# bootphon/shennong

Hardware: AMD Instinct MI355X
Metric: frames/s (25 ms/10 ms, 16 kHz) for fbank-40 + MFCC-13 at 1/2/4/8 GPUs (higher is better)
Workload: dtype f32

## Files before the change

### include/shennong_amd.h

```cpp
#ifndef SHENNONG_AMD_H_
#define SHENNONG_AMD_H_

#include <stdint.h>

#ifdef __cplusplus
extern "C" {
#endif

#define SNF_OK 0
#define SNF_E_INVALID (-1)
#define SNF_E_RUNTIME (-2)
#define SNF_E_HIP (-3)
#define SNF_E_NODEVICE (-4)

#define SNF_KIND_SPECTROGRAM 0
#define SNF_KIND_FBANK 1
#define SNF_KIND_MFCC 2
#define SNF_KIND_PLP 3
#define SNF_KIND_PITCH 4
#define SNF_KIND_PITCH_POST 5
#define SNF_KIND_DELTA 6
#define SNF_KIND_ENERGY 7
#define SNF_KIND_VAD 8
#define SNF_KIND_CMVN 9
// ... 295 lines not shown
int snf_memcpy_h2d_async(void* dst, const void* src, uint64_t bytes, void* stream);
int snf_memcpy_d2h_async(void* dst, const void* src, uint64_t bytes, void* stream);
int snf_event_create(void** event);
int snf_event_destroy(void* event);
int snf_event_record(void* event, void* stream);
int snf_event_synchronize(void* event);
int snf_stream_wait_event(void* stream, void* event);
int snf_event_elapsed_ms(void* start, void* stop, float* ms);
int snf_host_malloc(void** hptr, uint64_t bytes);
int snf_host_free(void* hptr);
int snf_wav_scan(const char* path, int32_t* channels, int32_t* sample_rate, int64_t* nsamples, int32_t* bits,
                 int32_t* format_tag);
int snf_wav_read_pcm16(const char* const* paths, int64_t n_files, const int64_t* first_sample,
                       const int64_t* n_samples, int16_t* dst, const int64_t* dst_offsets, int32_t threads,
                       int32_t* status);

#define SNF_COMM_ID_BYTES 128
typedef struct snf_comm snf_comm;
int snf_comm_unique_id(void* id128);
int snf_comm_init(const void* id128, int32_t world_size, int32_t rank, int32_t device_id, snf_comm** out);
int snf_comm_rank(const snf_comm* comm);
int snf_comm_world_size(const snf_comm* comm);
int snf_comm_destroy(snf_comm* comm);
int snf_comm_gatherv(snf_comm* comm, const float* d_send, int64_t send_count, float* d_recv,
                     const int64_t* recv_counts, int32_t root, void* stream);
int snf_comm_allreduce_f64(snf_comm* comm, double* d_buf, int64_t count, int32_t op, void* stream);

int snf_debug_fill_lds(uint32_t pattern);
int snf_debug_pitch_scratch(snf_plan* plan, void** down, void** nccf_res, void** pov_nccf,
                            void** states);
int snf_debug_plp_tail(snf_plan* plan, const float* mel, const double* energy,
                       const int64_t* frame_offsets, int64_t n_utts, float* out, float* mel_out);
int snf_debug_fbank512b_rel32(const int64_t* sample_offsets, const int64_t* frame_offsets, int64_t n_utts);
float snf_plan_last_kernel_ms(const snf_plan* plan, int which);
const char* snf_plan_kernel_name(const snf_plan* plan, int which);

#ifdef __cplusplus
}
#endif
#endif
```

### shennong_amd/_backend.py

```python

import ctypes as C
import os
import threading

import numpy as np

from shennong_amd import _abi

_HERE = os.path.dirname(os.path.abspath(__file__))
_LIB_PATH = os.environ.get('SHENNONG_AMD_LIB') or os.path.join(_HERE, 'libshennong_hip.so')
_LIB = None
_LOCK = threading.Lock()
_PLANS = {}
_DEVICE = int(os.environ.get('SHENNONG_AMD_DEVICE', '0'))

EXPORTS = [
    'snf_version', 'snf_last_error', 'snf_device_count', 'snf_set_device',
    'snf_device_name', 'snf_device_synchronize', 'snf_num_frames',
    'snf_first_sample_of_frame', 'snf_window_size', 'snf_window_shift',
    'snf_padded_window_size', 'snf_window_function', 'snf_pitch_num_frames',
    'snf_plan_create', 'snf_plan_destroy', 'snf_plan_ndims', 'snf_plan_fast_path',
    'snf_plan_num_frames', 'snf_plan_run_batch', 'snf_plan_run_batch_device',
    'snf_post_ndims', 'snf_post_run_batch', 'snf_post_run_batch_device',
    'snf_cmvn_accumulate', 'snf_cmvn_apply', 'snf_cmvn_accumulate_device',
    'snf_cmvn_apply_device', 'snf_concat_columns_device', 'snf_count_nonfinite_device', 'snf_set_noise_call',
    'snf_malloc', 'snf_free', 'snf_memcpy_h2d', 'snf_memcpy_d2h', 'snf_memset',
    'snf_host_malloc', 'snf_host_free', 'snf_debug_fill_lds', 'snf_debug_pitch_scratch',
    'snf_debug_plp_tail', 'snf_debug_fbank512b_rel32',
    'snf_stream_create', 'snf_stream_destroy', 'snf_stream_synchronize', 'snf_memcpy_h2d_async',
    'snf_memcpy_d2h_async', 'snf_comm_unique_id', 'snf_comm_init', 'snf_comm_rank', 'snf_comm_world_size',
    'snf_comm_destroy', 'snf_comm_gatherv', 'snf_comm_allreduce_f64',
    'snf_plan_last_kernel_ms', 'snf_plan_kernel_name', 'snf_set_oom_hook',
    'snf_event_create', 'snf_event_destroy', 'snf_event_record', 'snf_event_elapsed_ms', 'snf_mem_info',
    'snf_stream_wait_event', 'snf_stream_query', 'snf_event_synchronize', 'snf_wav_scan', 'snf_wav_read_pcm16',
    'snf_gmm_loglikes', 'snf_gmm_accumulate', 'snf_gmm_gselect', 'snf_gmm_gselect_preselect',
    'snf_gmm_selection_posteriors', 'snf_fmllr_accumulate', 'snf_vtln_gram', 'snf_lvtln_select',
    'snf_affine_apply_segments', 'snf_vtln_gram_rows', 'snf_dense_layer', 'snf_bottleneck_vad',
    'snf_bottleneck_fbank', 'snf_bottleneck_nn_input', 'snf_bottleneck_forward', 'snf_crepe_conv',
    'snf_crepe_forward', 'snf_crepe_decode', 'snf_framed_onehot', 'snf_packed_weights_bf16_size',
    'snf_pack_weights_bf16', 'snf_dense_layer_bf16', 'snf_bottleneck_forward_bf16', 'snf_crepe_conv_bf16',
    'snf_crepe_forward_bf16', 'snf_resample_num_out', 'snf_linear_resample', 'snf_crepe_rows',
    'snf_crepe_voicing_convert', 'snf_bottleneck_extract', 'snf_bottleneck_extract_runs',
    'snf_collate_num_out', 'snf_collate_padded', 'snf_dtw_pairs']


_OOM_HOOK_TYPE = C.CFUNCTYPE(None)


def _release_pool():
    try:
        DEVICE_POOL.clear()
    except Exception:
        pass


_OOM_HOOK = _OOM_HOOK_TYPE(_release_pool)


def lib():
    global _LIB
    if _LIB is not None:
# ... 34 lines not shown
        L.snf_plan_fast_path.argtypes = [vp]
        L.snf_plan_num_frames.argtypes = [vp, i64]
        L.snf_plan_num_frames.restype = i64
        L.snf_plan_run_batch.argtypes = [vp, pi16, pi64, i64, pf, pf, pi64]
        L.snf_plan_run_batch_device.argtypes = [
            vp, vp, pi64, i64, pf, vp, pi64, vp]
        L.snf_post_ndims.argtypes = [vp, i32]
        L.snf_post_run_batch.argtypes = [vp, pf, i32, pi64, i64, pf]
        L.snf_post_run_batch_device.argtypes = [vp, vp, i32, pi64, i64, vp, vp]
        pi32, pf64 = C.POINTER(C.c_int32), C.POINTER(C.c_double)
        L.snf_cmvn_accumulate.argtypes = [
            vp, pf, i32, pi64, i64, pf, pi32, i32, pf64]
        L.snf_cmvn_apply.argtypes = [
            vp, pf, i32, pi64, i64, pf64, pi32, i32, i32, i32, pf]
        L.snf_cmvn_accumulate_device.argtypes = [
            vp, vp, i32, pi64, i64, vp, pi32, i32, pf64]
        L.snf_cmvn_apply_device.argtypes = [
            vp, vp, i32, pi64, i64, pf64, pi32, i32, i32, i32, vp]
        L.snf_concat_columns_device.argtypes = [
            i32, vp, i32, pi64, vp, i32, pi64, i64, vp, pi64]
        L.snf_count_nonfinite_device.argtypes = [i32, vp, C.c_uint64, C.POINTER(C.c_uint64)]
        L.snf_set_noise_call.argtypes = [C.c_uint64]
        L.snf_malloc.argtypes = [C.POINTER(vp), C.c_uint64]
        L.snf_free.argtypes = [vp]
        L.snf_memcpy_h2d.argtypes = [vp, vp, C.c_uint64]
        L.snf_memcpy_d2h.argtypes = [vp, vp, C.c_uint64]
        L.snf_memset.argtypes = [vp, i32, C.c_uint64]
        L.snf_host_malloc.argtypes = [C.POINTER(vp), C.c_uint64]
        L.snf_host_free.argtypes = [vp]
        L.snf_debug_fill_lds.argtypes = [C.c_uint32]
        L.snf_debug_pitch_scratch.argtypes = [vp] + [C.POINTER(vp)] * 4
        L.snf_debug_plp_tail.argtypes = [vp, pf, C.POINTER(C.c_double), pi64, i64, pf, pf]
        L.snf_debug_fbank512b_rel32.argtypes = [pi64, pi64, i64]
        L.snf_stream_create.argtypes = [C.POINTER(vp)]
        L.snf_stream_destroy.argtypes = [vp]
        L.snf_stream_synchronize.argtypes = [vp]
        L.snf_stream_query.argtypes = [vp]
        L.snf_memcpy_h2d_async.argtypes = [vp, vp, C.c_uint64, vp]
        L.snf_event_create.argtypes = [C.POINTER(vp)]
        L.snf_event_destroy.argtypes = [vp]
        L.snf_event_record.argtypes = [vp, vp]
        L.snf_stream_wait_event.argtypes = [vp, vp]
        L.snf_event_synchronize.argtypes = [vp]
        L.snf_event_elapsed_ms.argtypes = [vp, vp, C.POINTER(C.c_float)]
        L.snf_memcpy_d2h_async.argtypes = [vp, vp, C.c_uint64, vp]
        L.snf_comm_unique_id.argtypes = [vp]
        L.snf_comm_init.argtypes = [vp, i32, i32, i32, C.POINTER(vp)]
        L.snf_comm_rank.argtypes = [vp]
        L.snf_comm_world_size.argtypes = [vp]
        L.snf_comm_destroy.argtypes = [vp]
        L.snf_comm_gatherv.argtypes = [vp, vp, i64, vp, pi64, i32, vp]
        L.snf_comm_allreduce_f64.argtypes = [vp, vp, i64, i32, vp]
        L.snf_plan_last_kernel_ms.argtypes = [vp, i32]
        L.snf_plan_last_kernel_ms.restype = f32
        L.snf_plan_kernel_name.argtypes = [vp, i32]
        L.snf_plan_kernel_name.restype = C.c_char_p
        L.snf_set_oom_hook.argtypes = [_OOM_HOOK_TYPE]
        L.snf_mem_info.argtypes = [C.POINTER(C.c_uint64), C.POINTER(C.c_uint64)]
        L.snf_wav_scan.argtypes = [C.c_char_p, pi32, pi32, pi64, pi32, pi32]
        L.snf_wav_read_pcm16.argtypes = [C.POINTER(C.c_char_p), i64, pi64, pi64, pi16, pi64, i32, pi32]
        L.snf_gmm_loglikes.argtypes = [i32, vp, i64, i32, vp, vp, vp, i32, vp, vp]
        L.snf_gmm_accumulate.argtypes = [i32, vp, i64, i32, vp, vp, vp, vp, i32, vp, vp, vp, vp]
        L.snf_gmm_gselect.argtypes = [i32, vp, i64, i32, vp, vp, vp, i32, i32, vp, vp, vp]
        L.snf_gmm_gselect_preselect.argtypes = [i32, vp, i64, i32, vp, vp, vp, i32, vp, i32, i32, vp, vp, vp]
        L.snf_gmm_selection_posteriors.argtypes = [i32, vp, i64, i32, vp, vp, vp, i32, vp, i32, f32, vp, vp, vp]
        L.snf_fmllr_accumulate.argtypes = [i32, vp, i64, i32, vp, vp, i32, vp, vp, i32, vp, i64, vp, vp]
# ... 1251 lines not shown
```

### shennong_amd/csrc/capi_mel.hip

```cpp
#include "plan.h"

using namespace snf;

namespace {

constexpr float kPairSplitRatio = 8.0f;

int check_offsets(const snf_plan* plan, const int64_t* sample_offsets, const int64_t* frame_offsets,
                  int64_t n_utts) {
  if (sample_offsets[0] != 0 || frame_offsets[0] != 0)
    return set_error(SNF_E_INVALID, "offsets tables must start at 0");
  for (int64_t u = 0; u < n_utts; ++u) {
    const int64_t n = sample_offsets[u + 1] - sample_offsets[u];
    const int64_t f = frame_offsets[u + 1] - frame_offsets[u];
    if (n < 0 || f < 0) return set_error(SNF_E_INVALID, "offsets tables must be non-decreasing");
    if (f != snf_plan_num_frames(plan, n))
      return set_error(SNF_E_INVALID, "frame_offsets do not match snf_plan_num_frames for utterance " +
                                          std::to_string(u));
  }
  return SNF_OK;
}

int run_pitch_device(snf_plan* plan, const int16_t* d_wave, const int64_t* sample_offsets,
                     int64_t n_utts, float* d_out, const int64_t* frame_offsets, hipStream_t s) {
// ... 446 lines not shown
  const size_t nb = static_cast<size_t>(plan->o.mel.num_bins), nc = static_cast<size_t>(plan->ndims);
  DevBuf d_mel, d_energy, d_foff, d_out;
  if ((rc = d_mel.ensure(sizeof(float) * nf * nb))) return rc;
  if ((rc = d_energy.ensure(sizeof(double) * nf))) return rc;
  if ((rc = d_out.ensure(sizeof(float) * nf * nc))) return rc;
  if ((rc = d_foff.upload(std::vector<int64_t>(frame_offsets, frame_offsets + n_utts + 1), s))) return rc;
  SNF_HIP_CHECK(hipMemcpyAsync(d_mel.p, mel, sizeof(float) * nf * nb, hipMemcpyHostToDevice, s));
  SNF_HIP_CHECK(hipMemcpyAsync(d_energy.p, energy, sizeof(double) * nf, hipMemcpyHostToDevice, s));
  BatchArgs b{};
  b.frame_offsets = d_foff.as<int64_t>();
  b.n_utts = n_utts;
  b.total_frames = total_frames;
  begin_timing(plan);
  if (plan->o.rasta) {
    if ((rc = launch_rasta(d_mel.as<float>(), b, static_cast<int>(nb), s))) return rc;
    mark_kernel(plan, "rasta_kernel");
  }
  const char* launched = nullptr;
  rc = launch_plp_tail(plan->pp, b, d_mel.as<float>(), d_energy.as<double>(), d_out.as<float>(), s, &launched);
  if (!rc && launched) mark_kernel(plan, launched);
  if (!rc) {
    SNF_HIP_CHECK(hipMemcpyAsync(out, d_out.p, sizeof(float) * nf * nc, hipMemcpyDeviceToHost, s));
    if (mel_out) SNF_HIP_CHECK(hipMemcpyAsync(mel_out, d_mel.p, sizeof(float) * nf * nb, hipMemcpyDeviceToHost, s));
  }
  SNF_HIP_CHECK(hipStreamSynchronize(s));
  return rc;
}

int snf_debug_fbank512b_rel32(const int64_t* sample_offsets, const int64_t* frame_offsets, int64_t n_utts) {
  if (!sample_offsets || !frame_offsets || n_utts < 0) return set_error(SNF_E_INVALID, "null offsets table");
  return fbank512b_rel32_ok(sample_offsets, frame_offsets, n_utts) ? 1 : 0;
}

}
```

### shennong_amd/csrc/device_fft.h

```cpp
#ifndef SNF_DEVICE_FFT_H_
#define SNF_DEVICE_FFT_H_

#include <float.h>
#include <hip/hip_runtime.h>

#include <cstdint>

namespace snf {

namespace {

__device__ __forceinline__ float fast_log(float x) {
  return __builtin_amdgcn_logf(x) * 0.69314718055994530942f;
}
__device__ __forceinline__ float floor_eps(float x) {
  return __builtin_amdgcn_fmed3f(x, FLT_EPSILON, FLT_MAX);
}
template <int SHIFT>
__device__ __forceinline__ void fmac_row_shl(float& acc, float src, float f) {
  asm volatile("s_nop 1\n v_fmac_f32_dpp %0, %1, %2 row_shl:%3 row_mask:0xf bank_mask:0xf bound_ctrl:1"
               : "+v"(acc) : "v"(src), "v"(f), "n"(SHIFT));
}

typedef __attribute__((address_space(3))) const void* lds_cptr;
__device__ __forceinline__ unsigned lds_addr(const void* p) {
  return static_cast<unsigned>(reinterpret_cast<uintptr_t>((lds_cptr)p));
}
__device__ __forceinline__ void lds_wait() {
  asm volatile("s_waitcnt lgkmcnt(0)" ::: "memory");
  __builtin_amdgcn_sched_barrier(0);
}
__device__ __forceinline__ void read16_b64(const void* base, float2 (&d)[16]) {
  asm volatile(
      "ds_read_b64 %0, %16\n ds_read_b64 %1, %16 offset:8\n ds_read_b64 %2, %16 offset:16\n"
      "ds_read_b64 %3, %16 offset:24\n ds_read_b64 %4, %16 offset:32\n ds_read_b64 %5, %16 offset:40\n"
      "ds_read_b64 %6, %16 offset:48\n ds_read_b64 %7, %16 offset:56\n ds_read_b64 %8, %16 offset:64\n"
      "ds_read_b64 %9, %16 offset:72\n ds_read_b64 %10, %16 offset:80\n ds_read_b64 %11, %16 offset:88\n"
      "ds_read_b64 %12, %16 offset:96\n ds_read_b64 %13, %16 offset:104\n ds_read_b64 %14, %16 offset:112\n"
      "ds_read_b64 %15, %16 offset:120\n s_waitcnt lgkmcnt(0)"
      : "=&v"(d[0]), "=&v"(d[1]), "=&v"(d[2]), "=&v"(d[3]), "=&v"(d[4]), "=&v"(d[5]), "=&v"(d[6]),
        "=&v"(d[7]), "=&v"(d[8]), "=&v"(d[9]), "=&v"(d[10]), "=&v"(d[11]), "=&v"(d[12]), "=&v"(d[13]),
        "=&v"(d[14]), "=&v"(d[15])
      : "v"(lds_addr(base))
      : "memory");
}
__device__ __forceinline__ void read_tw8_row16(const void* tw, const void* base, float4 (&q)[8], float2 (&d)[16]) {
  asm volatile(
      "ds_read_b128 %0, %24\n ds_read_b128 %1, %24 offset:16\n ds_read_b128 %2, %24 offset:32\n"
      "ds_read_b128 %3, %24 offset:48\n ds_read_b128 %4, %24 offset:64\n ds_read_b128 %5, %24 offset:80\n"
      "ds_read_b128 %6, %24 offset:96\n ds_read_b128 %7, %24 offset:112\n"
      "ds_read_b64 %8, %25\n ds_read_b64 %9, %25 offset:8\n ds_read_b64 %10, %25 offset:16\n"
      "ds_read_b64 %11, %25 offset:24\n ds_read_b64 %12, %25 offset:32\n ds_read_b64 %13, %25 offset:40\n"
      "ds_read_b64 %14, %25 offset:48\n ds_read_b64 %15, %25 offset:56\n ds_read_b64 %16, %25 offset:64\n"
      "ds_read_b64 %17, %25 offset:72\n ds_read_b64 %18, %25 offset:80\n ds_read_b64 %19, %25 offset:88\n"
// ... 303 lines not shown
```

### shennong_amd/csrc/kernels_fbank512b.hip

```cpp
#include <float.h>

#include <cstdlib>
#include <type_traits>

#include "snf_internal.h"
#include "device_fft.h"

namespace snf {

namespace {

typedef unsigned u32x4 __attribute__((ext_vector_type(4)));
typedef unsigned u32x2 __attribute__((ext_vector_type(2)));

constexpr int kWaves = kFast512MaxWaves;
constexpr int kHeaderFloats = kFast512HeaderFloats;
constexpr int kTileRow = kFast512TileRow;
constexpr int kTileBytes = kFast512TileBytes;


}

template <int NJ, int KIND, int ENERGY, bool BST, bool DITHER, int MMQ, int LV, bool REL>
__global__ __launch_bounds__(kWaves * 64, 4) void fbank512b_kernel(const Fast512Params p, const BatchArgs b,
// ... 17 lines not shown
  float2* tile = reinterpret_cast<float2*>(wave_base);
  float* ptile = reinterpret_cast<float*>(wave_base) + q * 16;
  tile[l * kTileRow + 16] = make_float2(0.0f, 0.0f);
  const int mj = lane & 3;
  const float* __restrict__ mm_lane = tab + p.off_mm_lane + lane;
  const float* __restrict__ mtile =
      reinterpret_cast<const float*>(smem + tab_bytes + (wid * 4 + mj) * kTileBytes) + mj * 16;
  int mm_start_once = 0, mm_out_once = 0;
  if (NJ == 13) {
    mm_start_once = reinterpret_cast<const int*>(mm_lane)[0];
    mm_out_once = reinterpret_cast<const int*>(mm_lane)[64];
  }
  static_assert(MMQ == 0 || (NJ == 13 && (MMQ == 6 || MMQ == 7) && (LV == 3 || LV == 4)), "plans of launch_plan");
  const float4* __restrict__ mm_b_once = reinterpret_cast<const float4*>(mtile + mm_start_once);
  float lifter_once = 1.0f;
  if (NJ == 13 && KIND == SNF_KIND_MFCC) lifter_once = t_lifter[l];

  const float win_len_f = static_cast<float>(p.win_len), inv_win_len = 1.0f / win_len_f;
  using idx_t = typename std::conditional<REL, int, int64_t>::type;
  const idx_t total_frames = static_cast<idx_t>(b.total_frames);
  const idx_t n_sets = (total_frames + 3) >> 2;
  const idx_t set_stride = static_cast<idx_t>(gridDim.x) * kWaves;
  const idx_t last_frame = total_frames - 1;
  idx_t set = static_cast<idx_t>(blockIdx.x) * kWaves + wid;
  if (set >= n_sets) return;

  const bool in_last = 2 * (l + 16 * (NJ - 1)) < p.win_len;
  auto in_window = [&](int j) -> bool {
    if (NJ == 13) return j < NJ - 1 || in_last;
    return 2 * (l + 16 * j) < p.win_len;
  };
  static_assert(!REL || NJ == 13, "set-relative addressing: the 25 ms forms");
  const unsigned q8 = static_cast<unsigned>(q) * 8u;
  auto set_rows_of = [&](const void* table, idx_t s) -> uint64_t {
    int rows = static_cast<int>(total_frames) - static_cast<int>(s) * 4;
    rows = rows < 0 ? 0 : rows;
    asm volatile("" : "+s"(rows));
    rows = rows > 4 ? 4 : rows;
    const __amdgpu_buffer_rsrc_t rsrc = __builtin_amdgcn_make_buffer_rsrc(
        const_cast<char*>(static_cast<const char*>(table)) + static_cast<int64_t>(s) * 32, 0, rows * 8, 0x00020000);
    const u32x2 v = __builtin_amdgcn_raw_buffer_load_b64(rsrc, q8, 0, 0);
    return (static_cast<uint64_t>(v.y) << 32) | v.x;
  };
  auto start_of = [&](idx_t s) -> int64_t {
    if (REL) return static_cast<int64_t>(set_rows_of(b.frame_start, s));
    const int64_t gi = s * 4 + q;
    return b.frame_start[gi < last_frame ? gi : last_frame];
  };
  auto noise_of = [&](idx_t s) -> unsigned long long {
    if (!DITHER) return 0ull;
    if (REL) return set_rows_of(b.frame_noise, s);
    const int64_t gi = s * 4 + q;
    return b.frame_noise[gi < last_frame ? gi : last_frame];
  };
  typedef int __attribute__((aligned(2))) int_a2;
  int raw[NJ];
  const unsigned l4 = 4u * l, off12 = in_last ? l4 + 64u * 12u : 0u;
  auto request = [&](int64_t st) {
    if (REL) {
      const unsigned lo = static_cast<unsigned>(st), hi = static_cast<unsigned>(static_cast<uint64_t>(st) >> 32);
      const unsigned lo0 = __builtin_amdgcn_readfirstlane(lo), hi0 = __builtin_amdgcn_readfirstlane(hi);
      const int64_t st0 = static_cast<int64_t>((static_cast<uint64_t>(hi0) << 32) | lo0);
      const int64_t left = b.rel32_samples - st0;
      unsigned over = static_cast<unsigned>(static_cast<uint64_t>(left) >> 31);
      asm volatile("" : "+s"(over));
      const __amdgpu_buffer_rsrc_t wrsrc = __builtin_amdgcn_make_buffer_rsrc(
          const_cast<int16_t*>(b.wave + st0), 0, over != 0u ? -1 : static_cast<int>(static_cast<unsigned>(left) << 1),
          0x00020000);
      unsigned off = ((lo - lo0) << 1) + l4, last = ((lo - lo0) << 1) + off12;
      asm volatile("" : "+v"(off), "+v"(last));
#pragma unroll
      for (int j = 0; j < NJ - 1; ++j)
        raw[j] = static_cast<int>(__builtin_amdgcn_raw_buffer_load_b32(wrsrc, off + 64u * j, 0, 0));
      raw[NJ - 1] = static_cast<int>(__builtin_amdgcn_raw_buffer_load_b32(wrsrc, last, 0, 0));
      return;
    }
    const int16_t* __restrict__ wp = b.wave + st;
    const int16_t* __restrict__ wl = wp + 2 * l;
#pragma unroll
    for (int j = 0; j < NJ; ++j)
      raw[j] = *reinterpret_cast<const int_a2*>((NJ == 13 && j < NJ - 1) || in_window(j) ? wl + 32 * j : wp);
  };
  float4 w512q[4];
  read_quads<4>(t_tw512 + l * 10, w512q);
  int64_t start_next = start_of(set + set_stride);
  unsigned long long noise_cur = noise_of(set), noise_next = noise_of(set + set_stride);
  request(start_of(set));
  if (BST) {
    const __amdgpu_buffer_rsrc_t none = __builtin_amdgcn_make_buffer_rsrc(out, 0, 0, 0x00020000);
    if (KIND == SNF_KIND_MFCC) __builtin_amdgcn_raw_buffer_store_b32(0u, none, -1, 0, 0);
    else __builtin_amdgcn_raw_buffer_store_b128(u32x4{0u, 0u, 0u, 0u}, none, -1, 0, 2);
  }

  for (; set < n_sets; set += set_stride) {
    const idx_t g = set * 4 + q;
    const bool valid = g <= last_frame;

    float xe[NJ], xo[NJ];
    int part_i = 0;
    float part = 0.0f;
    unsigned dkey_lo = 0, dkey_hi = 0;
    if (DITHER) {
      const unsigned long long k = noise_cur ^ p.seed;
      dkey_lo = fmix32(static_cast<unsigned>(k));
      dkey_hi = fmix32(static_cast<unsigned>(k >> 32) ^ dkey_lo);
      asm volatile("" : "+v"(dkey_lo), "+v"(dkey_hi));
    }
    const float dscale = DITHER ? dither_scale(p.dither) : 0.0f;
#pragma unroll
    for (int j = 0; j < NJ; ++j) {
      xe[j] = static_cast<float>(static_cast<short>(raw[j] & 0xffff));
      xo[j] = static_cast<float>(raw[j] >> 16);
      if (DITHER) {
        add_dither_pair(dkey_lo, dkey_hi, static_cast<unsigned>(l + 16 * j), dscale, xe[j], xo[j]);
        const float s2 = xe[j] + xo[j];
        part += in_window(j) ? s2 : 0.0f;
      } else {
        const int both = __builtin_amdgcn_sdot2(__builtin_bit_cast(short2v, raw[j]), short2v{1, 1}, part_i, false);
        part_i = in_window(j) ? both : part_i;
      }
    }
    if (!DITHER) part = static_cast<float>(part_i);
#pragma unroll
    for (int j = 0; j < NJ; ++j) asm volatile("" : "+v"(xe[j]), "+v"(xo[j]) : : "memory");
    asm volatile("" : "+v"(part) : : "memory");
    request(start_next);
    start_next = start_of(set + 2 * set_stride);
    if (DITHER) {
      noise_cur = noise_next;
      noise_next = noise_of(set + 2 * set_stride);
    }

    float neg_mean = 0.0f;
    if (p.remove_dc) {
      const float sum = row_sum16(part);
      const float qv = sum * inv_win_len;
      neg_mean = -__builtin_fmaf(__builtin_fmaf(-qv, win_len_f, sum), inv_win_len, qv);
      if (DITHER) neg_mean = -sum / win_len_f;
    }
    float2 z[16];
    float e_raw = 0.0f, e_post = 0.0f;
    float rot_prev = xe[0] + neg_mean;
    float left[13];
    if (NJ == 13) {
#pragma unroll
      for (int j = 0; j < 13; ++j) left[j] = dpp_row_ror<0x121>(xo[j] + neg_mean);
      row_head_carry13(left, rot_prev, 0x0001000100010001ull);
    }
#pragma unroll
    for (int jj = 0; jj < 16; jj += 2) {
      float4 w4;
      if (jj < NJ)
        w4 = *reinterpret_cast<const float4*>(__builtin_assume_aligned(t_win + l * 18 + jj, 16));
#pragma unroll
      for (int j = jj; j < jj + 2; ++j) {
        if (j < NJ) {
          const float ae = xe[j] + neg_mean, ao = xo[j] + neg_mean;
          float ap;
          if (NJ == 13) {
            ap = left[j < 13 ? j : 0];
          } else {
            const float rot = dpp_row_ror<0x121>(ao);
            ap = l == 0 ? rot_prev : rot;
// ... 76 lines not shown
      const unsigned pk_addr = lds_addr(ptile + l), pm_addr = lds_addr(ptile + (144 - l));
#define SNF_W2(ADDR_, A_, B_, O0_, O1_) \
  asm volatile("ds_write2_b32 %0, %1, %2 offset0:" #O0_ " offset1:" #O1_ : : "v"(ADDR_), "v"(A_), "v"(B_) : "memory")
      SNF_W2(pk_addr, pk[0], pk[1], 0, 16);
      SNF_W2(pk_addr, pk[2], pk[3], 32, 48);
      SNF_W2(pk_addr, pk[4], pk[5], 64, 80);
      SNF_W2(pk_addr, pk[6], pk[7], 96, 112);
      SNF_W2(pm_addr, pm[7], pm[6], 0, 16);
      SNF_W2(pm_addr, pm[5], pm[4], 32, 48);
      SNF_W2(pm_addr, pm[3], pm[2], 64, 80);
      SNF_W2(pm_addr, pm[1], pm[0], 96, 112);
#undef SNF_W2
      if (l == 0) ptile[128] = p128;
    }
    wave_lds_order();
    __builtin_amdgcn_sched_barrier(0);
    float4 mm_x[7];
    if (MMQ != 0) {
      issue_quads<MMQ, 1>(mm_b_once, mm_x);
      __builtin_amdgcn_sched_barrier(0);
    }

    float log_energy = 0.0f;
    if (ENERGY != 0) {
      if (KIND == SNF_KIND_PLP) {
        if (valid && l == 0) energy_out[g] = static_cast<double>(e_lin);
      } else {
        log_energy = fast_log(floor_eps(e_lin));
        if (p.has_floor && log_energy < p.log_energy_floor) log_energy = p.log_energy_floor;
      }
    }
    float* __restrict__ row = out + g * static_cast<int64_t>(p.out_cols);
    const idx_t rows_left = total_frames - set * 4;
    const __amdgpu_buffer_rsrc_t orsrc = __builtin_amdgcn_make_buffer_rsrc(
        out + static_cast<int64_t>(set) * 4 * static_cast<int64_t>(p.out_cols), 0,
        (rows_left < 4 ? static_cast<int>(rows_left) : 4) * p.out_cols * 4, 0x00020000);
    {
      const bool mvalid = set * 4 + mj <= last_frame;
      const int mm_start = NJ == 13 ? mm_start_once : reinterpret_cast<const int*>(mm_lane)[0];
      const float4* __restrict__ bsrc = reinterpret_cast<const float4*>(mtile + mm_start);
      const float4* __restrict__ asrc = t_mm_a + lane;
      f32x4 acc0 = {0.0f, 0.0f, 0.0f, 0.0f}, acc1 = {0.0f, 0.0f, 0.0f, 0.0f};
#define SNF_QUAD(A_, X_)                                                   \
  do {                                                                     \
    acc0 = __builtin_amdgcn_mfma_f32_4x4x1f32(A_.x, X_.x, acc0, 0, 0, 0);   \
    acc1 = __builtin_amdgcn_mfma_f32_4x4x1f32(A_.y, X_.y, acc1, 0, 0, 0);   \
    acc0 = __builtin_amdgcn_mfma_f32_4x4x1f32(A_.z, X_.z, acc0, 0, 0, 0);   \
    acc1 = __builtin_amdgcn_mfma_f32_4x4x1f32(A_.w, X_.w, acc1, 0, 0, 0);   \
  } while (0)
      const int n_quads = p.mm_quads;
      if (MMQ != 0) {
        land_quad(mm_x[MMQ - 1]);
#pragma unroll
        for (int t = 0; t < MMQ; ++t) SNF_QUAD(mm_w[t], mm_x[t]);
      } else if (n_quads == 7 || n_quads == 6) {
        float4 a[7], x[7];
#pragma unroll
        for (int t = 0; t < 7; ++t) {
          a[t] = asrc[t * 64];
          x[t] = bsrc[t];
        }
#pragma unroll
        for (int t = 0; t < 7; ++t)
          if (t < 6 || n_quads == 7) SNF_QUAD(a[t], x[t]);
      } else {
        float4 a0 = asrc[0], x0 = bsrc[0];
        int t = 0;
        for (; t + 1 < n_quads; t += 2) {
          const float4 a1 = asrc[(t + 1) * 64], x1 = bsrc[t + 1];
          SNF_QUAD(a0, x0);
          a0 = asrc[(t + 2) * 64];
          x0 = bsrc[t + 2];
          SNF_QUAD(a1, x1);
        }
        if (t < n_quads) SNF_QUAD(a0, x0);
      }
#undef SNF_QUAD
      float mel[4];
#pragma unroll
      for (int i = 0; i < 4; ++i) mel[i] = acc0[i] + acc1[i];
      const int mm_out = NJ == 13 ? mm_out_once : reinterpret_cast<const int*>(mm_lane)[64];
      if (LV == 4) {
#pragma unroll
        for (int i = 0; i < 4; ++i) {
          const float own = mel[i];
          fmac_row_shl<4>(mel[i], own, mm_f[0]);
          fmac_row_shl<8>(mel[i], own, mm_f[1]);
          fmac_row_shl<12>(mel[i], own, mm_f[2]);
        }
      } else if (LV == 3) {
#pragma unroll
        for (int i = 0; i < 4; ++i) {
          const float own = mel[i];
          fmac_row_shl<4>(mel[i], own, mm_f[0]);
          fmac_row_shl<8>(mel[i], own, mm_f[1]);
        }
      } else if (p.mm_levels > 1) {
        const float mm_f1 = mm_lane[128], mm_f2 = mm_lane[192], mm_f3 = mm_lane[256];
        if (p.mm_levels > 3) {
#pragma unroll
          for (int i = 0; i < 4; ++i) {
            const float own = mel[i];
            fmac_row_shl<4>(mel[i], own, mm_f1);
            fmac_row_shl<8>(mel[i], own, mm_f2);
            fmac_row_shl<12>(mel[i], own, mm_f3);
          }
        } else {
#pragma unroll
          for (int i = 0; i < 4; ++i) {
            const float own = mel[i];
            fmac_row_shl<4>(mel[i], own, mm_f1);
            fmac_row_shl<8>(mel[i], own, mm_f2);
          }
        }
      }
      const int mel_col = (KIND == SNF_KIND_FBANK && p.use_energy && !p.htk_compat) ? 1 : 0;
      if (KIND == SNF_KIND_FBANK || KIND == SNF_KIND_PLP) {
        if (KIND == SNF_KIND_FBANK && p.use_log) {
#pragma unroll
          for (int i = 0; i < 4; ++i) mel[i] = fast_log(floor_eps(mel[i]));
        }
        if (BST) {
          __builtin_amdgcn_raw_buffer_store_b128(
              __builtin_bit_cast(u32x4, f32x4{mel[0], mel[1], mel[2], mel[3]}), orsrc,
              mm_out >= 0 ? (mj * p.out_cols + mm_out) * 4 : -1, 0, 2);
        } else {
          if (mvalid && mm_out >= 0) {
            float* __restrict__ dst = out + static_cast<int64_t>(set * 4 + mj) * p.out_cols + mel_col + mm_out;
            if (mm_out + 4 <= p.num_bins) {
// ... 46 lines not shown
            v += w[g4].x * x[g4].x;
            v += w[g4].y * x[g4].y;
            v += w[g4].z * x[g4].z;
            v += w[g4].w * x[g4].w;
          }
        } else {
          write_log_mel();
#pragma unroll 2
          for (int g4 = 0; g4 < p.dd_groups; ++g4) {
            const float4 w = dw[g4 * 16], x = dx[g4];
            v += w.x * x.x;
            v += w.y * x.y;
            v += w.z * x.z;
            v += w.w * x.w;
          }
        }
        v *= NJ == 13 ? lifter_once : t_lifter[l];
        if (l == 0 && p.use_energy) v = log_energy;
        int oc = l;
        if (p.htk_compat) {
          oc = l == 0 ? p.num_ceps - 1 : l - 1;
          if (l == 0 && !p.use_energy)
            v = static_cast<float>(static_cast<double>(v) * 1.4142135623730950488016887);
        }
        if (BST) {
          __builtin_amdgcn_raw_buffer_store_b32(__builtin_bit_cast(unsigned, v), orsrc,
                                                l < p.num_ceps ? (q * p.out_cols + oc) * 4 : -1, 0, 0);
        } else if (valid && l < p.num_ceps) {
          row[oc] = v;
        }
      }
    }
    wave_lds_order();
  }
}

bool fbank512b_shape_ok(const Fast512Params& p, bool per_utt) {
  if (const char* knob = getenv("SNF_FBANK512_OLD"))
    if (knob[0] == '1') return false;
  if (p.dual || p.fused_delta || per_utt) return false;
  if (!p.snip_edges || p.dct_mfma) return false;
  if (p.kind != SNF_KIND_FBANK && p.kind != SNF_KIND_MFCC && p.kind != SNF_KIND_PLP) return false;
  return fast512_lds_bytes(p.table_floats, kWaves, false) <= kFast512LdsBytes;
}
bool fbank512b_rel32_spans_ok(const int64_t* sample_offsets, const int64_t* frame_offsets, int64_t n_utts) {
  constexpr int64_t kLimit = int64_t{1} << 30;
  if (frame_offsets[n_utts] >= kLimit) return false;
  int64_t first[3];
  int held = 0;
  for (int64_t u = 0; u < n_utts; ++u) {
    if (frame_offsets[u + 1] == frame_offsets[u]) continue;
    if (held == 3) {
      if (sample_offsets[u] - first[0] >= kLimit) return false;
      first[0] = first[1];
      first[1] = first[2];
      --held;
    }
    first[held++] = sample_offsets[u];
  }
  return held == 0 || sample_offsets[n_utts] - first[0] < kLimit;
}
bool fbank512b_addr64_knob() {
  const char* knob = getenv("SNF_FBANK512B_ADDR64");
  return knob && knob[0] == '1';
}
bool fbank512b_rel32_ok(const int64_t* sample_offsets, const int64_t* frame_offsets, int64_t n_utts) {
  return !fbank512b_addr64_knob() && fbank512b_rel32_spans_ok(sample_offsets, frame_offsets, n_utts);
}
bool fbank512b_eligible(const Fast512Params& p, const BatchArgs& b) {
  if (p.dither != 0.0f && b.frame_noise == nullptr) return false;
  return fbank512b_shape_ok(p, b.blk_utt != nullptr);
}

namespace {

template <int NJ, int KIND, int ENERGY, bool BST, bool DITHER, int MMQ, int LV, bool REL>
int launch_form(const Fast512Params& q, const BatchArgs& b, float* out, double* energy_out, hipStream_t stream) {
  const size_t lds = fast512_lds_bytes(q.table_floats, kWaves, false);
  const int64_t n_sets = (b.total_frames + 3) / 4;
  int64_t blocks = (n_sets + kWaves - 1) / kWaves;
  if (blocks > 256) blocks = 256;
  auto kern = fbank512b_kernel<NJ, KIND, ENERGY, BST, DITHER, MMQ, LV, REL>;
  if (lds > 64 * 1024)
    SNF_HIP_CHECK(hipFuncSetAttribute(reinterpret_cast<const void*>(kern),
                                      hipFuncAttributeMaxDynamicSharedMemorySize, static_cast<int>(lds)));
  hipLaunchKernelGGL(kern, dim3(static_cast<unsigned>(blocks)), dim3(kWaves * 64), lds, stream, q, b, out,
                     energy_out);
  SNF_HIP_CHECK(hipGetLastError());
  return SNF_OK;
}

template <int NJ, int KIND, int ENERGY, bool BST, bool DITHER, int MMQ, int LV>
int launch_dither(const Fast512Params& q, const BatchArgs& b, float* out, double* energy_out, hipStream_t stream) {
  if constexpr (NJ == 13 && !(KIND == SNF_KIND_MFCC && DITHER && MMQ == 7 && LV == 3)) {
    if (b.rel32_samples > 0)
      return launch_form<NJ, KIND, ENERGY, BST, DITHER, MMQ, LV, true>(q, b, out, energy_out, stream);
  }
  return launch_form<NJ, KIND, ENERGY, BST, DITHER, MMQ, LV, false>(q, b, out, energy_out, stream);
}

template <int NJ, int KIND, int ENERGY, bool BST, bool DITHER>
int launch_plan(const Fast512Params& q, const BatchArgs& b, float* out, double* energy_out, hipStream_t stream) {
  if constexpr (NJ == 13 && (BST || !DITHER)) {
    constexpr bool kFits74 = !(KIND == SNF_KIND_MFCC && DITHER && ENERGY != 0);
    if (q.mm_quads == 7 && q.mm_levels == 4) {
      if constexpr (kFits74)
        return launch_dither<NJ, KIND, ENERGY, BST, DITHER, 7, 4>(q, b, out, energy_out, stream);
      else
        return launch_dither<NJ, KIND, ENERGY, BST, DITHER, 0, 0>(q, b, out, energy_out, stream);
    }
    if (q.mm_quads == 7 && q.mm_levels >= 2)
      return launch_dither<NJ, KIND, ENERGY, BST, DITHER, 7, 3>(q, b, out, energy_out, stream);
    if (q.mm_quads == 6 && q.mm_levels == 4)
      return launch_dither<NJ, KIND, ENERGY, BST, DITHER, 6, 4>(q, b, out, energy_out, stream);
// ... 92 lines not shown
```

### shennong_amd/csrc/snf_internal.h

```cpp
#ifndef SNF_INTERNAL_H_
#define SNF_INTERNAL_H_

#include <hip/hip_runtime.h>
#include <stdint.h>

#include <map>
#include <mutex>
#include <string>
#include <vector>

#include "../../include/shennong_amd.h"

namespace snf {

int set_error(int code, const std::string& msg);
const char* last_error();

#define SNF_HIP_CHECK(expr)                                                                  \
  do {                                                                                       \
    hipError_t _e = (expr);                                                                  \
    if (_e != hipSuccess)                                                                    \
      return snf::set_error(SNF_E_HIP, std::string(#expr) + ": " + hipGetErrorString(_e));   \
  } while (0)

// ... 173 lines not shown
  int fused_delta;
  const float* delta_scales;
  int table_floats;
  int table_stride;
  const float* tables;
  int off_mm_a, off_mm_lane, off_dd_a, off_lifter, off_dd_v;
};

bool fast512_eligible(const MelParams& mp, bool any_warp);
bool fast512_dual_eligible(const MelParams& mp);
int fast512_build(const MelParams& mp, const std::vector<float>& window, const MelBanksHost& mb,
                  const std::vector<float>& dct, const std::vector<float>& lifter, bool dual,
                  std::vector<float>* blob, Fast512Params* out);
int launch_build_pair_table(const int64_t* d_frame_offsets, const int64_t* d_sample_offsets,
                            const int64_t* d_pair_offsets, int64_t n_utts, int64_t n_pairs, int win_shift,
                            int win_len, int snip_edges, PairRec* d_pairs, hipStream_t stream);
int launch_build_frame_start(const int64_t* d_frame_offsets, const int64_t* d_sample_offsets,
                             int64_t n_utts, int64_t total_frames, int64_t total_samples, int win_shift,
                             int win_len, int snip_edges, int64_t* d_frame_start, int32_t* d_frame_edge,
                             int32_t* d_frame_utt, hipStream_t stream);
int launch_fbank512(const Fast512Params& p, const BatchArgs& b, float* out, int out_cols,
                    double* energy_out, hipStream_t stream, const char** launched = nullptr);
int launch_fbank256x2(const Fast512Params& p, const BatchArgs& b, float* out, int out_cols,
                      double* energy_out, hipStream_t stream);
int launch_build_frame_noise(const BatchArgs& b, uint64_t* d_keys, hipStream_t stream);
int launch_build_utt_noise(const BatchArgs& b, uint32_t* d_words, hipStream_t stream);
bool fbank512b_eligible(const Fast512Params& p, const BatchArgs& b);
bool fbank512b_shape_ok(const Fast512Params& p, bool per_utt);
bool fbank512b_rel32_spans_ok(const int64_t* sample_offsets, const int64_t* frame_offsets, int64_t n_utts);
bool fbank512b_addr64_knob();
bool fbank512b_rel32_ok(const int64_t* sample_offsets, const int64_t* frame_offsets, int64_t n_utts);
int launch_fbank512b(const Fast512Params& p, const BatchArgs& b, float* out, int out_cols,
                     double* energy_out, hipStream_t stream);

bool fbank2048_eligible(const MelParams& mp);
void fbank2048_tables(const MelParams& mp, const std::vector<float>& window, std::vector<float>* blob);
int launch_fbank2048(const MelParams& p, const BatchArgs& b, const float* tables, float* out, int out_cols,
                     double* energy_out, hipStream_t stream);

bool fbank1024x2_eligible(const MelParams& mp);
void fbank1024x2_tables(const MelParams& mp, const std::vector<float>& window, std::vector<float>* blob);
int launch_fbank1024x2(const MelParams& p, const BatchArgs& b, const float* tables, float* out, int out_cols,
                       double* energy_out, hipStream_t stream);

int launch_mfcc_dct(const float* in, int in_cols, int num_bins, int num_ceps, const float* dct_t, const float* lifter,
                    int use_energy, int htk_compat, int64_t total_frames, float* out, int out_cols,
                    hipStream_t stream);

struct PitchDevTables {
  int first_lag, last_lag, num_lags, num_states, win_size, win_shift, full_len;
  int ar_max_taps, rs_in_unit, rs_out_unit, rs_max_taps;
  int snip_edges, recompute_frame;
  float soft_min_f0, inter_frame_factor, nccf_ballast;
  const float* lags;
  const int* ar_first;
  const int* ar_n;
  const float* ar_w;
  int ar_groups, ar_quad_taps;
  const float* ar_quad_w;
  const int* ar_quad_base;
  const int* rs_first;
  const int* rs_ntaps;
  const float* rs_w;
};
struct PitchBatch {
  const int16_t* wave;
// ... 200 lines not shown
```

Measured before the change: 3.270 billion.

## Add scalar cursor for set-relative fbank512b addressing and single-wait prefetch

Adds a scalar cursor struct that carries the look-ahead table address, output address and remaining rows across loop trips, so the set-relative kernel forms stop recomputing per-set 64-bit offsets and row clamps. It also reorders the prologue so the first frame request is issued before the next-set table loads, followed by one explicit waitcnt per trip, and batches the mel block-join DPP fmacs into one inline-asm block. A host debug entry point checks the cursor sequence. The costs are more template specialization, hand-tuned waitcnt immediates that depend on how many loads are outstanding, and asm that fixes instruction order.

```diff
diff --git a/include/shennong_amd.h b/include/shennong_amd.h
--- a/include/shennong_amd.h
+++ b/include/shennong_amd.h
@@ -351,6 +351,9 @@
 int snf_debug_plp_tail(snf_plan* plan, const float* mel, const double* energy,
                        const int64_t* frame_offsets, int64_t n_utts, float* out, float* mel_out);
 int snf_debug_fbank512b_rel32(const int64_t* sample_offsets, const int64_t* frame_offsets, int64_t n_utts);
+int64_t snf_debug_fbank512b_cursor(int64_t total_frames, int32_t out_cols, uint64_t table_base, uint64_t out_base,
+                                   int64_t first_set, int64_t max_trips, int64_t* set_stride, uint64_t* ahead_addr,
+                                   int32_t* ahead_rows, uint64_t* out_addr, int32_t* out_rows);
 float snf_plan_last_kernel_ms(const snf_plan* plan, int which);
 const char* snf_plan_kernel_name(const snf_plan* plan, int which);
 
diff --git a/shennong_amd/_backend.py b/shennong_amd/_backend.py
--- a/shennong_amd/_backend.py
+++ b/shennong_amd/_backend.py
@@ -26,7 +26,7 @@
     'snf_cmvn_apply_device', 'snf_concat_columns_device', 'snf_count_nonfinite_device', 'snf_set_noise_call',
     'snf_malloc', 'snf_free', 'snf_memcpy_h2d', 'snf_memcpy_d2h', 'snf_memset',
     'snf_host_malloc', 'snf_host_free', 'snf_debug_fill_lds', 'snf_debug_pitch_scratch',
-    'snf_debug_plp_tail', 'snf_debug_fbank512b_rel32',
+    'snf_debug_plp_tail', 'snf_debug_fbank512b_rel32', 'snf_debug_fbank512b_cursor',
     'snf_stream_create', 'snf_stream_destroy', 'snf_stream_synchronize', 'snf_memcpy_h2d_async',
     'snf_memcpy_d2h_async', 'snf_comm_unique_id', 'snf_comm_init', 'snf_comm_rank', 'snf_comm_world_size',
     'snf_comm_destroy', 'snf_comm_gatherv', 'snf_comm_allreduce_f64',
@@ -127,6 +127,10 @@
         L.snf_debug_pitch_scratch.argtypes = [vp] + [C.POINTER(vp)] * 4
         L.snf_debug_plp_tail.argtypes = [vp, pf, C.POINTER(C.c_double), pi64, i64, pf, pf]
         L.snf_debug_fbank512b_rel32.argtypes = [pi64, pi64, i64]
+        L.snf_debug_fbank512b_cursor.argtypes = [i64, C.c_int32, C.c_uint64, C.c_uint64, i64, i64, pi64,
+                                                 C.POINTER(C.c_uint64), C.POINTER(C.c_int32),
+                                                 C.POINTER(C.c_uint64), C.POINTER(C.c_int32)]
+        L.snf_debug_fbank512b_cursor.restype = i64
         L.snf_stream_create.argtypes = [C.POINTER(vp)]
         L.snf_stream_destroy.argtypes = [vp]
         L.snf_stream_synchronize.argtypes = [vp]
diff --git a/shennong_amd/csrc/capi_mel.hip b/shennong_amd/csrc/capi_mel.hip
--- a/shennong_amd/csrc/capi_mel.hip
+++ b/shennong_amd/csrc/capi_mel.hip
@@ -502,4 +502,27 @@
   return fbank512b_rel32_ok(sample_offsets, frame_offsets, n_utts) ? 1 : 0;
 }
 
-}
+int64_t snf_debug_fbank512b_cursor(int64_t total_frames, int32_t out_cols, uint64_t table_base, uint64_t out_base,
+                                   int64_t first_set, int64_t max_trips, int64_t* set_stride, uint64_t* ahead_addr,
+                                   int32_t* ahead_rows, uint64_t* out_addr, int32_t* out_rows) {
+  if (total_frames <= 0 || total_frames >= (int64_t{1} << 30) || out_cols <= 0)
+    return set_error(SNF_E_INVALID, "set-relative launches: 1 .. 2^30 - 1 frames");
+  const int64_t stride = fbank512b_grid_blocks(total_frames) * kFast512MaxWaves;
+  if (first_set < 0 || first_set >= stride || first_set >= (total_frames + 3) / 4)
+    return set_error(SNF_E_INVALID, "no wave of the launch starts at this frame set");
+  if (set_stride) *set_stride = stride;
+  Fbank512bCursor cur;
+  cur.init(table_base, table_base, out_base, static_cast<int>(total_frames), static_cast<int>(first_set),
+           static_cast<int>(stride), out_cols);
+  int64_t trips = 0;
+  for (; cur.rows > 0; cur.advance<false>(), ++trips) {
+    if (trips >= max_trips) continue;
+    if (ahead_addr) ahead_addr[trips] = cur.ahead;
+    if (ahead_rows) ahead_rows[trips] = cur.ahead_rows();
+    if (out_addr) out_addr[trips] = cur.out;
+    if (out_rows) out_rows[trips] = cur.out_rows();
+  }
+  return trips;
+}
+
+}
diff --git a/shennong_amd/csrc/device_fft.h b/shennong_amd/csrc/device_fft.h
--- a/shennong_amd/csrc/device_fft.h
+++ b/shennong_amd/csrc/device_fft.h
@@ -20,6 +20,31 @@
 __device__ __forceinline__ void fmac_row_shl(float& acc, float src, float f) {
   asm volatile("s_nop 1\n v_fmac_f32_dpp %0, %1, %2 row_shl:%3 row_mask:0xf bank_mask:0xf bound_ctrl:1"
                : "+v"(acc) : "v"(src), "v"(f), "n"(SHIFT));
+}
+template <int LV>
+__device__ __forceinline__ void join_row_blocks(float (&acc)[4], const float (&f)[3]) {
+  static_assert(LV == 3 || LV == 4, "two or three neighbouring blocks to add");
+  float o0, o1, o2, o3;
+#define SNF_JOIN(SH_, F_)                                                                        \
+  "v_fmac_f32_dpp %0, %4, " F_ " row_shl:" #SH_ " row_mask:0xf bank_mask:0xf bound_ctrl:1\n"     \
+  "v_fmac_f32_dpp %1, %5, " F_ " row_shl:" #SH_ " row_mask:0xf bank_mask:0xf bound_ctrl:1\n"     \
+  "v_fmac_f32_dpp %2, %6, " F_ " row_shl:" #SH_ " row_mask:0xf bank_mask:0xf bound_ctrl:1\n"     \
+  "v_fmac_f32_dpp %3, %7, " F_ " row_shl:" #SH_ " row_mask:0xf bank_mask:0xf bound_ctrl:1\n"
+#define SNF_JOIN_COPY "v_mov_b32 %0, %4\n v_mov_b32 %1, %5\n v_mov_b32 %2, %6\n v_mov_b32 %3, %7\n"
+  if (LV == 4)
+    asm volatile(SNF_JOIN_COPY SNF_JOIN(4, "%8") SNF_JOIN(8, "%9") SNF_JOIN(12, "%10")
+                 : "=&v"(o0), "=&v"(o1), "=&v"(o2), "=&v"(o3)
+                 : "v"(acc[0]), "v"(acc[1]), "v"(acc[2]), "v"(acc[3]), "v"(f[0]), "v"(f[1]), "v"(f[2]));
+  else
+    asm volatile(SNF_JOIN_COPY SNF_JOIN(4, "%8") SNF_JOIN(8, "%9")
+                 : "=&v"(o0), "=&v"(o1), "=&v"(o2), "=&v"(o3)
+                 : "v"(acc[0]), "v"(acc[1]), "v"(acc[2]), "v"(acc[3]), "v"(f[0]), "v"(f[1]));
+#undef SNF_JOIN_COPY
+#undef SNF_JOIN
+  acc[0] = o0;
+  acc[1] = o1;
+  acc[2] = o2;
+  acc[3] = o3;
 }
 
 typedef __attribute__((address_space(3))) const void* lds_cptr;
diff --git a/shennong_amd/csrc/kernels_fbank512b.hip b/shennong_amd/csrc/kernels_fbank512b.hip
--- a/shennong_amd/csrc/kernels_fbank512b.hip
+++ b/shennong_amd/csrc/kernels_fbank512b.hip
@@ -73,15 +73,18 @@
   };
   static_assert(!REL || NJ == 13, "set-relative addressing: the 25 ms forms");
   const unsigned q8 = static_cast<unsigned>(q) * 8u;
+  auto rows_at = [&](uint64_t first_row, int rows) -> uint64_t {
+    const __amdgpu_buffer_rsrc_t rsrc =
+        __builtin_amdgcn_make_buffer_rsrc(reinterpret_cast<char*>(first_row), 0, rows * 8, 0x00020000);
+    const u32x2 v = __builtin_amdgcn_raw_buffer_load_b64(rsrc, q8, 0, 0);
+    return (static_cast<uint64_t>(v.y) << 32) | v.x;
+  };
   auto set_rows_of = [&](const void* table, idx_t s) -> uint64_t {
     int rows = static_cast<int>(total_frames) - static_cast<int>(s) * 4;
     rows = rows < 0 ? 0 : rows;
     asm volatile("" : "+s"(rows));
     rows = rows > 4 ? 4 : rows;
-    const __amdgpu_buffer_rsrc_t rsrc = __builtin_amdgcn_make_buffer_rsrc(
-        const_cast<char*>(static_cast<const char*>(table)) + static_cast<int64_t>(s) * 32, 0, rows * 8, 0x00020000);
-    const u32x2 v = __builtin_amdgcn_raw_buffer_load_b64(rsrc, q8, 0, 0);
-    return (static_cast<uint64_t>(v.y) << 32) | v.x;
+    return rows_at(reinterpret_cast<uint64_t>(table) + static_cast<uint64_t>(static_cast<int64_t>(s)) * 32u, rows);
   };
   auto start_of = [&](idx_t s) -> int64_t {
     if (REL) return static_cast<int64_t>(set_rows_of(b.frame_start, s));
@@ -124,18 +127,39 @@
   };
   float4 w512q[4];
   read_quads<4>(t_tw512 + l * 10, w512q);
-  int64_t start_next = start_of(set + set_stride);
-  unsigned long long noise_cur = noise_of(set), noise_next = noise_of(set + set_stride);
-  request(start_of(set));
+  constexpr bool kOneWait = NJ == 13 && BST && !(KIND == SNF_KIND_MFCC && DITHER && MMQ == 7 && !REL);
+  int64_t start_next = 0;
+  unsigned long long noise_cur = noise_of(set), noise_next = 0;
+  if (kOneWait) {
+    request(start_of(set));
+    __builtin_amdgcn_sched_barrier(0);
+    start_next = start_of(set + set_stride);
+    noise_next = noise_of(set + set_stride);
+    __builtin_amdgcn_sched_barrier(0);
+  } else {
+    start_next = start_of(set + set_stride);
+    noise_next = noise_of(set + set_stride);
+    request(start_of(set));
+  }
+  constexpr bool kCursor = REL && !(KIND == SNF_KIND_MFCC && !BST && MMQ == 7);
+  Fbank512bCursor cur;
+  if (kCursor)
+    cur.init(reinterpret_cast<uint64_t>(b.frame_start), reinterpret_cast<uint64_t>(b.frame_noise),
+             reinterpret_cast<uint64_t>(out), static_cast<int>(total_frames), static_cast<int>(set),
+             static_cast<int>(set_stride), p.out_cols);
   if (BST) {
     const __amdgpu_buffer_rsrc_t none = __builtin_amdgcn_make_buffer_rsrc(out, 0, 0, 0x00020000);
     if (KIND == SNF_KIND_MFCC) __builtin_amdgcn_raw_buffer_store_b32(0u, none, -1, 0, 0);
     else __builtin_amdgcn_raw_buffer_store_b128(u32x4{0u, 0u, 0u, 0u}, none, -1, 0, 2);
   }
 
-  for (; set < n_sets; set += set_stride) {
+  for (; kCursor ? cur.rows > 0 : set < n_sets; set += set_stride) {
     const idx_t g = set * 4 + q;
     const bool valid = g <= last_frame;
+    if (kOneWait) {
+      __builtin_amdgcn_s_waitcnt(0x0F70 | (DITHER ? 3 : 2));
+      __builtin_amdgcn_sched_barrier(0);
+    }
 
     float xe[NJ], xo[NJ];
     int part_i = 0;
@@ -166,10 +190,19 @@
     for (int j = 0; j < NJ; ++j) asm volatile("" : "+v"(xe[j]), "+v"(xo[j]) : : "memory");
     asm volatile("" : "+v"(part) : : "memory");
     request(start_next);
-    start_next = start_of(set + 2 * set_stride);
-    if (DITHER) {
-      noise_cur = noise_next;
-      noise_next = noise_of(set + 2 * set_stride);
+    if (kCursor) {
+      const int ahead_rows = cur.ahead_rows();
+      start_next = static_cast<int64_t>(rows_at(cur.ahead, ahead_rows));
+      if (DITHER) {
+        noise_cur = noise_next;
+        noise_next = rows_at(cur.noise, ahead_rows);
+      }
+    } else {
+      start_next = start_of(set + 2 * set_stride);
+      if (DITHER) {
+        noise_cur = noise_next;
+        noise_next = noise_of(set + 2 * set_stride);
+      }
     }
 
     float neg_mean = 0.0f;
@@ -312,9 +345,12 @@
     }
     float* __restrict__ row = out + g * static_cast<int64_t>(p.out_cols);
     const idx_t rows_left = total_frames - set * 4;
-    const __amdgpu_buffer_rsrc_t orsrc = __builtin_amdgcn_make_buffer_rsrc(
-        out + static_cast<int64_t>(set) * 4 * static_cast<int64_t>(p.out_cols), 0,
-        (rows_left < 4 ? static_cast<int>(rows_left) : 4) * p.out_cols * 4, 0x00020000);
+    const __amdgpu_buffer_rsrc_t orsrc =
+        kCursor ? __builtin_amdgcn_make_buffer_rsrc(reinterpret_cast<char*>(cur.out), 0,
+                                                    cur.out_rows() * (p.out_cols * 4), 0x00020000)
+                : __builtin_amdgcn_make_buffer_rsrc(
+                      out + static_cast<int64_t>(set) * 4 * static_cast<int64_t>(p.out_cols), 0,
+                      (rows_left < 4 ? static_cast<int>(rows_left) : 4) * p.out_cols * 4, 0x00020000);
     {
       const bool mvalid = set * 4 + mj <= last_frame;
       const int mm_start = NJ == 13 ? mm_start_once : reinterpret_cast<const int*>(mm_lane)[0];
@@ -361,20 +397,9 @@
       for (int i = 0; i < 4; ++i) mel[i] = acc0[i] + acc1[i];
       const int mm_out = NJ == 13 ? mm_out_once : reinterpret_cast<const int*>(mm_lane)[64];
       if (LV == 4) {
-#pragma unroll
-        for (int i = 0; i < 4; ++i) {
-          const float own = mel[i];
-          fmac_row_shl<4>(mel[i], own, mm_f[0]);
-          fmac_row_shl<8>(mel[i], own, mm_f[1]);
-          fmac_row_shl<12>(mel[i], own, mm_f[2]);
-        }
+        join_row_blocks<4>(mel, mm_f);
       } else if (LV == 3) {
-#pragma unroll
-        for (int i = 0; i < 4; ++i) {
-          const float own = mel[i];
-          fmac_row_shl<4>(mel[i], own, mm_f[0]);
-          fmac_row_shl<8>(mel[i], own, mm_f[1]);
-        }
+        join_row_blocks<3>(mel, mm_f);
       } else if (p.mm_levels > 1) {
         const float mm_f1 = mm_lane[128], mm_f2 = mm_lane[192], mm_f3 = mm_lane[256];
         if (p.mm_levels > 3) {
@@ -487,6 +512,7 @@
       }
     }
     wave_lds_order();
+    if (kCursor) cur.template advance<DITHER>();
   }
 }
 
@@ -532,9 +558,7 @@
 template <int NJ, int KIND, int ENERGY, bool BST, bool DITHER, int MMQ, int LV, bool REL>
 int launch_form(const Fast512Params& q, const BatchArgs& b, float* out, double* energy_out, hipStream_t stream) {
   const size_t lds = fast512_lds_bytes(q.table_floats, kWaves, false);
-  const int64_t n_sets = (b.total_frames + 3) / 4;
-  int64_t blocks = (n_sets + kWaves - 1) / kWaves;
-  if (blocks > 256) blocks = 256;
+  const int64_t blocks = fbank512b_grid_blocks(b.total_frames);
   auto kern = fbank512b_kernel<NJ, KIND, ENERGY, BST, DITHER, MMQ, LV, REL>;
   if (lds > 64 * 1024)
     SNF_HIP_CHECK(hipFuncSetAttribute(reinterpret_cast<const void*>(kern),
diff --git a/shennong_amd/csrc/snf_internal.h b/shennong_amd/csrc/snf_internal.h
--- a/shennong_amd/csrc/snf_internal.h
+++ b/shennong_amd/csrc/snf_internal.h
@@ -229,6 +229,56 @@
 bool fbank512b_rel32_ok(const int64_t* sample_offsets, const int64_t* frame_offsets, int64_t n_utts);
 int launch_fbank512b(const Fast512Params& p, const BatchArgs& b, float* out, int out_cols,
                      double* energy_out, hipStream_t stream);
+inline int64_t fbank512b_grid_blocks(int64_t total_frames) {
+  const int64_t n_sets = (total_frames + 3) / 4;
+  const int64_t blocks = (n_sets + kFast512MaxWaves - 1) / kFast512MaxWaves;
+  return blocks > 256 ? 256 : blocks;
+}
+#if defined(__HIP_DEVICE_COMPILE__)
+#define SNF_PIN_SCALAR(x) asm volatile("" : "+s"(x))
+#else
+#define SNF_PIN_SCALAR(x) (void)(x)
+#endif
+struct Fbank512bCursor {
+  uint64_t ahead;
+  uint64_t noise;
+  uint64_t out;
+  int rows;
+  uint64_t ahead_step, out_step;
+  int rows_step, rows_ahead;
+  __host__ __device__ __forceinline__ void init(uint64_t starts, uint64_t keys, uint64_t out_base, int total_frames,
+                                                int set, int set_stride, int out_cols) {
+    const uint64_t first = (static_cast<uint64_t>(set) + 2u * static_cast<uint64_t>(set_stride)) * 32u;
+    ahead = starts + first;
+    noise = keys + first;
+    out = out_base + static_cast<uint64_t>(set) * 16u * static_cast<uint64_t>(out_cols);
+    rows = total_frames - set * 4;
+    ahead_step = static_cast<uint64_t>(set_stride) * 32u;
+    out_step = static_cast<uint64_t>(set_stride) * 16u * static_cast<uint64_t>(out_cols);
+    rows_step = set_stride * 4;
+    rows_ahead = set_stride * 8;
+  }
+  __host__ __device__ __forceinline__ int ahead_rows() const {
+    int r = rows - rows_ahead;
+    r = r < 0 ? 0 : r;
+    SNF_PIN_SCALAR(r);
+    return r > 4 ? 4 : r;
+  }
+  __host__ __device__ __forceinline__ int out_rows() const { return rows < 4 ? rows : 4; }
+  template <bool WITH_NOISE>
+  __host__ __device__ __forceinline__ void advance() {
+    ahead += ahead_step;
+    out += out_step;
+    rows -= rows_step;
+    SNF_PIN_SCALAR(ahead);
+    SNF_PIN_SCALAR(out);
+    SNF_PIN_SCALAR(rows);
+    if (WITH_NOISE) {
+      noise += ahead_step;
+      SNF_PIN_SCALAR(noise);
+    }
+  }
+};
 
 bool fbank2048_eligible(const MelParams& mp);
 void fbank2048_tables(const MelParams& mp, const std::vector<float>& window, std::vector<float>* blob);
```

New measurement: 3.288 billion (median of 6 runs). About the same (+0.6%).
